# janelia-flyem/transfer_em

Hardware: AMD Instinct MI355X
Metric: CycleGAN train steps/sec on 132^3 x1 uint8 volumes (per-GPU batch of 1 volume; aggregate over GPUs) (higher is better)
Workload: dtype f32

## Files before the change

include/tem_hip.h:

```cpp
#ifndef TEM_HIP_H
#define TEM_HIP_H

#include <stdint.h>

#ifdef __cplusplus
extern "C" {
#endif

#define TEM_ABI_VERSION 1

#define TEM_OK            0
#define TEM_EINVAL       -1
#define TEM_EUNSUPPORTED -2
#define TEM_ESHAPE       -3

typedef void *tem_stream_t;

typedef struct tem_view {
  float  *ptr;
  int32_t N, D, H, W, C;
  int64_t sN, sD, sH, sW;
} tem_view;

typedef struct tem_epilogue {
// ... 94 lines not shown
int tem_adam_keras(float *theta, const float *grad, float *m, float *v, int64_t n,
                   float lr, float beta1, float beta2, float eps, float grad_scale,
                   const uint32_t *step_dev, tem_stream_t stream);

int tem_step_tick(uint32_t *step_dev, tem_stream_t stream);

int tem_dropout_masks(uint8_t *mask0, int64_t nbytes0, uint32_t site0, uint8_t *mask1, int64_t nbytes1, uint32_t site1,
                      uint64_t seed, const uint32_t *step_dev, uint32_t step, tem_stream_t stream);

int tem_u8_to_f32_std(const uint8_t *in, float *out, int64_t n, float mean, float std,
                      tem_stream_t stream);

int tem_f32_unstd_to_u8(const tem_view *y, uint8_t *out, int64_t oD, int64_t oH, int64_t oW,
                        float mean, float std, tem_stream_t stream);

int tem_u8_tiles_to_f32_std(const uint8_t *vol, int32_t Z, int32_t Y, int32_t X, const int32_t *origins_dev,
                            int32_t ntile, int32_t edge, float *out, float mean, float std, tem_stream_t stream);

int tem_f32_tiles_unstd_to_u8(const float *y, int32_t ntile, int32_t yedge, int32_t tpad, const int32_t *index_dev,
                              uint8_t *out, int32_t OZ, int32_t OY, int32_t OX, float mean, float std,
                              tem_stream_t stream);

int tem_augment_f32(const float *src, int32_t D, int32_t H, int32_t W, int32_t p0, int32_t p1, int32_t p2,
                    int32_t f0, int32_t f1, int32_t f2, float scale, float shift, float *dst, tem_stream_t stream);

int tem_warp_f32(const float *src, int32_t D, int32_t H, int32_t W, float rate, uint64_t seed, float *dst,
                 uint8_t *seeds, double *sum, tem_stream_t stream);

int tem_fill_f32(float *dst, int64_t n, float value, tem_stream_t stream);

int tem_copy_view(const tem_view *src, const tem_view *dst, tem_stream_t stream);

int tem_add_view(const tem_view *src, const tem_view *dst, tem_stream_t stream);

typedef struct tem_wlayer {
  int64_t offset;
  int32_t ntap, ci, co;
} tem_wlayer;

int tem_flip_transpose(const float *theta, float *theta_t, const tem_wlayer *layers_dev, int32_t nlayers,
                       int64_t total, tem_stream_t stream);

typedef struct tem_wino_layer {
  int64_t src_off, dst_off;
  int32_t ci, co, flip;
} tem_wino_layer;

int tem_winograd_weights(const float *theta, float *u, const tem_wino_layer *layers_dev, int32_t nlayers,
                         tem_stream_t stream);

int tem_conv_bwd_weight_winograd_nslab(const tem_bww_args *a, char *name, int32_t name_len);
int tem_conv_bwd_weight_winograd(const tem_bww_args *a, tem_stream_t stream);

int tem_leaky_gate_view(const tem_view *g, const tem_view *saved, float slope, tem_stream_t stream);

int tem_conv_bf16(const tem_conv_args *a, tem_stream_t stream);

int tem_conv_bf16_describe(const tem_conv_args *a, char *name, int32_t name_len);

int tem_conv_transpose_bf16(const tem_conv_args *a, tem_stream_t stream);
int tem_conv_transpose_bf16_describe(const tem_conv_args *a, char *name, int32_t name_len);

int tem_conv_bwd_weight_bf16(const tem_bww_args *a, tem_stream_t stream);
int tem_conv_bwd_weight_bf16_nslab(const tem_bww_args *a, char *name, int32_t name_len);

int tem_cast_f32_to_bf16(const float *src, void *dst, int64_t n, tem_stream_t stream);

int tem_pack_weights_bf16(const float *theta, void *theta_h, void *theta_ht, const tem_wlayer *layers_dev,
                          int32_t nlayers, int64_t total, tem_stream_t stream);

int tem_focal_logits_bf16(const tem_view *z, int32_t target, float gamma, double *losses, uint32_t slot_mask,
                          float loss_scale, const tem_view *dz, float grad_scale, tem_stream_t stream);
int tem_focal_match_bf16(const tem_view *a, const tem_view *b, float gamma, double *losses, uint32_t slot_mask,
                         float loss_scale, const tem_view *db, float grad_scale, tem_stream_t stream);
int tem_copy_view_bf16(const tem_view *src, const tem_view *dst, tem_stream_t stream);
int tem_add_view_bf16(const tem_view *src, const tem_view *dst, tem_stream_t stream);
int tem_channel_sum_bf16(const tem_view *g, float *out, int32_t accumulate, tem_stream_t stream);

int tem_instance_norm(const tem_view *x, const float *scale, const float *offset, float eps,
                      const tem_view *y, float *mean, float *rstd, tem_stream_t stream);

int tem_instance_norm_bwd(const tem_view *x, const tem_view *dy, const float *scale, const float *mean,
                          const float *rstd, const tem_view *dx, float *dscale, float *doffset,
                          double *workspace, tem_stream_t stream);

int tem_abi_version(const char **arch);

#ifdef __cplusplus
}
#endif
#endif
```

transfer_em_amd/_lib.py:

```python
import ctypes as C
import os

import torch

_HERE = os.path.dirname(os.path.abspath(__file__))
LIB_PATH = os.path.join(_HERE, "lib", "libtem_hip.so")

TEM_OK, TEM_EINVAL, TEM_EUNSUPPORTED, TEM_ESHAPE = 0, -1, -2, -3
TEM_W_TAP_CI_CO, TEM_W_FLIP_CO_CI, TEM_W_WINOGRAD = 0, 1, 2
_ERR = {TEM_EINVAL: "TEM_EINVAL (malformed descriptor)",
        TEM_EUNSUPPORTED: "TEM_EUNSUPPORTED (geometry outside the compiled set)",
        TEM_ESHAPE: "TEM_ESHAPE (inconsistent tensor extents)"}


class TemError(RuntimeError):
    pass


class tem_view(C.Structure):
    _fields_ = [("ptr", C.c_void_p),
                ("N", C.c_int32), ("D", C.c_int32), ("H", C.c_int32), ("W", C.c_int32), ("C", C.c_int32),
                ("sN", C.c_int64), ("sD", C.c_int64), ("sH", C.c_int64), ("sW", C.c_int64)]


# ... 40 lines not shown

_VP = C.POINTER(tem_view)
_SIGS = {
    "tem_disc_head_nslab": [C.c_int64],
    "tem_disc_head_fwd": [C.c_void_p, C.c_void_p, C.c_void_p, C.c_void_p, C.c_void_p, C.c_void_p, C.c_int64, C.c_float, C.c_void_p],
    "tem_disc_head_bwd": [C.POINTER(tem_head_bwd_args), C.c_void_p],
    "tem_conv": [C.POINTER(tem_conv_args), C.c_void_p],
    "tem_conv_transpose": [C.POINTER(tem_conv_args), C.c_void_p],
    "tem_conv_direct": [C.POINTER(tem_conv_args), C.c_void_p],
    "tem_conv_transpose_direct": [C.POINTER(tem_conv_args), C.c_void_p],
    "tem_conv_bf16": [C.POINTER(tem_conv_args), C.c_void_p],
    "tem_conv_bf16_describe": [C.POINTER(tem_conv_args), C.c_char_p, C.c_int32],
    "tem_conv_transpose_bf16": [C.POINTER(tem_conv_args), C.c_void_p],
    "tem_conv_transpose_bf16_describe": [C.POINTER(tem_conv_args), C.c_char_p, C.c_int32],
    "tem_conv_bwd_weight_bf16": [C.POINTER(tem_bww_args), C.c_void_p],
    "tem_conv_bwd_weight_bf16_nslab": [C.POINTER(tem_bww_args), C.c_char_p, C.c_int32],
    "tem_cast_f32_to_bf16": [C.c_void_p, C.c_void_p, C.c_int64, C.c_void_p],
    "tem_pack_weights_bf16": [C.c_void_p, C.c_void_p, C.c_void_p, C.c_void_p, C.c_int32, C.c_int64, C.c_void_p],
    "tem_focal_logits_bf16": [_VP, C.c_int32, C.c_float, C.c_void_p, C.c_uint32, C.c_float, _VP, C.c_float, C.c_void_p],
    "tem_focal_match_bf16": [_VP, _VP, C.c_float, C.c_void_p, C.c_uint32, C.c_float, _VP, C.c_float, C.c_void_p],
    "tem_copy_view_bf16": [_VP, _VP, C.c_void_p],
    "tem_add_view_bf16": [_VP, _VP, C.c_void_p],
    "tem_channel_sum_bf16": [_VP, C.c_void_p, C.c_int32, C.c_void_p],
    "tem_conv_is_tiled": [C.POINTER(tem_conv_args), C.c_int32, C.c_char_p, C.c_int32],
    "tem_bww_is_tiled": [C.POINTER(tem_bww_args), C.c_char_p, C.c_int32],
    "tem_conv_bwd_weight": [C.POINTER(tem_bww_args), C.c_void_p],
    "tem_conv_bwd_weight_nslab": [C.POINTER(tem_bww_args)],
    "tem_reduce_slabs": [C.c_void_p, C.c_int32, C.c_int64, C.c_int64, C.c_void_p, C.c_int32, C.c_float, C.c_void_p],
    "tem_reduce_slabs_multi": [C.c_void_p, C.c_int32, C.c_float, C.c_void_p],
    "tem_channel_sum": [_VP, C.c_void_p, C.c_int32, C.c_void_p],
    "tem_focal_logits": [_VP, C.c_int32, C.c_float, C.c_void_p, C.c_uint32, C.c_float, _VP, C.c_float, C.c_void_p],
    "tem_focal_match": [_VP, _VP, C.c_float, C.c_void_p, C.c_uint32, C.c_float, _VP, C.c_float, C.c_void_p],
    "tem_adam_keras": [C.c_void_p, C.c_void_p, C.c_void_p, C.c_void_p, C.c_int64, C.c_float, C.c_float, C.c_float,
                       C.c_float, C.c_float, C.c_void_p, C.c_void_p],
    "tem_step_tick": [C.c_void_p, C.c_void_p],
    "tem_dropout_masks": [C.c_void_p, C.c_int64, C.c_uint32, C.c_void_p, C.c_int64, C.c_uint32, C.c_uint64, C.c_void_p,
                          C.c_uint32, C.c_void_p],
    "tem_u8_to_f32_std": [C.c_void_p, C.c_void_p, C.c_int64, C.c_float, C.c_float, C.c_void_p],
    "tem_f32_unstd_to_u8": [_VP, C.c_void_p, C.c_int64, C.c_int64, C.c_int64, C.c_float, C.c_float, C.c_void_p],
    "tem_u8_tiles_to_f32_std": [C.c_void_p, C.c_int32, C.c_int32, C.c_int32, C.c_void_p, C.c_int32, C.c_int32, C.c_void_p,
                                C.c_float, C.c_float, C.c_void_p],
    "tem_f32_tiles_unstd_to_u8": [C.c_void_p, C.c_int32, C.c_int32, C.c_int32, C.c_void_p, C.c_void_p, C.c_int32, C.c_int32,
                                  C.c_int32, C.c_float, C.c_float, C.c_void_p],
    "tem_augment_f32": [C.c_void_p, C.c_int32, C.c_int32, C.c_int32, C.c_int32, C.c_int32, C.c_int32, C.c_int32, C.c_int32,
                        C.c_int32, C.c_float, C.c_float, C.c_void_p, C.c_void_p],
    "tem_warp_f32": [C.c_void_p, C.c_int32, C.c_int32, C.c_int32, C.c_float, C.c_uint64, C.c_void_p, C.c_void_p, C.c_void_p,
                     C.c_void_p],
    "tem_fill_f32": [C.c_void_p, C.c_int64, C.c_float, C.c_void_p],
    "tem_copy_view": [_VP, _VP, C.c_void_p],
    "tem_add_view": [_VP, _VP, C.c_void_p],
    "tem_leaky_gate_view": [_VP, _VP, C.c_float, C.c_void_p],
    "tem_flip_transpose": [C.c_void_p, C.c_void_p, C.c_void_p, C.c_int32, C.c_int64, C.c_void_p],
    "tem_conv_bwd_weight_winograd_nslab": [C.POINTER(tem_bww_args), C.c_char_p, C.c_int32],
    "tem_conv_bwd_weight_winograd": [C.POINTER(tem_bww_args), C.c_void_p],
    "tem_winograd_weights": [C.c_void_p, C.c_void_p, C.c_void_p, C.c_int32, C.c_void_p],
    "tem_instance_norm": [_VP, C.c_void_p, C.c_void_p, C.c_float, _VP, C.c_void_p, C.c_void_p, C.c_void_p],
    "tem_instance_norm_bwd": [_VP, _VP, C.c_void_p, C.c_void_p, C.c_void_p, _VP, C.c_void_p, C.c_void_p, C.c_void_p,
                              C.c_void_p],
    "tem_abi_version": [C.POINTER(C.c_char_p)],
}
EXPORTS = tuple(_SIGS)

_lib = None


def load():
    global _lib
    if _lib is not None:
        return _lib
    if not os.path.exists(LIB_PATH):
        raise TemError(
            f"{LIB_PATH} not found: the HIP extension is not built. Run `python -c 'import __graft_entry__ as g; "
            "g.build()'` (or `python -m transfer_em_amd.build`). transfer_em_amd has no CPU fallback.")
    lib = C.CDLL(LIB_PATH)
    for name, argtypes in _SIGS.items():
        try:
            fn = getattr(lib, name)
        except AttributeError as e:
            raise TemError(f"libtem_hip.so does not export {name}; rebuild it") from e
        fn.argtypes = argtypes
        fn.restype = C.c_int
    _lib = lib
    return lib


def check(rc, what):
    if rc != 0:
        msg = _ERR.get(rc, f"hipError {rc}")
        raise TemError(f"{what}: {msg}")
```

transfer_em_amd/csrc/wino.hip:

```cpp
#include "tem_common.h"
#include "wino_common.h"
#include <cmath>
#include <cstdio>
#include <cstdlib>

namespace wino {

#ifdef TEM_DEBUG_KNOBS
#define KDBG(x) (x)
#else
#define KDBG(x) 0
#endif


struct Ep32 {
  float slope;
  const float *gate; int32_t gN, gD, gH, gW; float gate_slope;
  const uint8_t *keep_mask;
  int32_t doz, doy, dox, dD, dH, dW;
  int32_t gbytes, mbytes;
};

struct Dev {
  const float *in0, *in1;
  int32_t i0N, i0D, i0H, i0W, i1N, i1D, i1H, i1W;
  int32_t C0;
  int32_t N, D, H, W;
  const float *u;
  float *out0, *out1;
  int32_t o0N, o0D, o0H, o0W, o1N, o1D, o1H, o1W;
  int32_t CO0;
  int32_t OD, OH, OW;
  int32_t P;
  int32_t BY, BX, nby, nbx, zsegs, zper, NTZ;
  int32_t E, PLC, subb, slotb;
  int32_t ndma;
  int32_t span0, span1;
  uint32_t magicBX, magicE;
  int32_t dbg;
  int32_t obytes;
  unsigned long long *stamps;
  Ep32 ep;
};

template <int CI, int CO, int NI, int EP, int EE>
__global__ __launch_bounds__(512) void wino_conv_k(Dev p) {
  constexpr int NH = CI / 8, VB = 32;
  constexpr int NB = (CO + 15) / 16;
  constexpr bool STREAM = CI == 32;
  constexpr bool PAIR = CI == 8 && CO == 8;
  constexpr int NKZ = PAIR ? 4 : 3;
  constexpr int UCH = 2 * NB * 16 * 128;
  extern __shared__ __attribute__((aligned(16))) float lds[];
  char *const ring = reinterpret_cast<char *>(lds);
  const int tid = threadIdx.x, lane = tid & 63;
  const int wave = __builtin_amdgcn_readfirstlane(tid >> 6);
  const int m = lane & 15, q = lane >> 4;
  const int grp = PAIR ? wave : (NB == 1 ? wave >> 1 : wave >> 2);
  const int nb = NB == 1 ? 0 : (wave >> 1) & 1;
  const int zb = PAIR ? (q >> 1) : (wave & 1);
  const int co = PAIR ? 4 * (q & 1) : nb * 16 + 4 * q;
  float *const uld = reinterpret_cast<float *>(ring + 4 * p.slotb);

  int seg = (int)xcd_contiguous_block(blockIdx.x, gridDim.x);
  const int zseg = seg % p.zsegs; seg /= p.zsegs;
  const int bx = seg % p.nbx; seg /= p.nbx;
  const int by = seg % p.nby;
  const int n = seg / p.nby;
  const int tz0 = zseg * p.zper, tz1 = min(p.NTZ, tz0 + p.zper), nsteps = tz1 - tz0;
  const int oy0 = by * 2 * p.BY, ox0 = bx * 2 * p.BX;
  const int ntile = p.BY * p.BX;

  const bool two_in = p.in1 != p.in0;
  const float *const in0n = p.in0 + (size_t)n * p.i0N, *const in1n = p.in1 + (size_t)n * p.i1N;
  int voff0[NI], voff1[NI];
  {
    const int iy0 = oy0 - p.P, ix0 = ox0 - p.P;
#pragma unroll
    for (int i = 0; i < NI; ++i) {
      const int sp = (wave + 8 * i) * 64 + lane;
      const bool ex = sp < p.PLC;
      const int spc = ex ? sp : 0;
      const int cpos = spc & 1, ve = spc >> 1;
      const int ro = ve / EE, e = ve - ro * EE;
      const int o = ro & 1, yr = ro >> 1;
      const int c = (cpos ^ swz(e, yr)) * 4;
      const int iy = iy0 + yr, ix = ix0 + 2 * e + o;
      const bool ok = ex && (unsigned)iy < (unsigned)p.H && (unsigned)ix < (unsigned)p.W;
      voff0[i] = ok ? (iy * p.i0H + ix * p.i0W + c) * 4 : (int)0x80000000;
      voff1[i] = ok ? (iy * p.i1H + ix * p.i1W + c) * 4 : (int)0x80000000;
      asm volatile("" : "+v"(voff0[i]), "+v"(voff1[i]));
    }
  }
  auto dma_plane = [&](int iz, int slot) {
    const bool zok = (unsigned)iz < (unsigned)p.D;
    const int izc = zok ? iz : 0;
#pragma unroll
    for (int h = 0; h < NH; ++h) {
      char *const dst = ring + slot * p.slotb + h * p.subb;
      if (!two_in || 8 * h < p.C0)
        dma_subimage<NI, !STREAM>(in0n + izc * p.i0D + 8 * h, zok ? p.span0 - 32 * h : 0, voff0, dst, wave, p.ndma);
      else
        dma_subimage<NI, !STREAM>(in1n + izc * p.i1D + (8 * h - p.C0), zok ? p.span1 - 4 * (8 * h - p.C0) : 0, voff1, dst, wave, p.ndma);
    }
  };

  const int izb0 = 2 * tz0 - p.P;
  if (nsteps > 0) {
#pragma unroll
    for (int k = 0; k < 4; ++k) dma_plane(izb0 + k, k);
  }
  auto dma_u = [&](int chunk, int buf) {
    const __amdgpu_buffer_rsrc_t r = __builtin_amdgcn_make_buffer_rsrc((void *)(p.u + (size_t)chunk * UCH), 0, UCH * 4, 0x00020000);
#pragma unroll
    for (int i = 0; i < UCH * 4 / 1024 / 8; ++i) {
      const int j = wave + 8 * i;
      __builtin_amdgcn_raw_ptr_buffer_load_lds(r, (__attribute__((address_space(3))) void *)((char *)uld + buf * (UCH * 4) + j * 1024), 16,
                                               (j * 64 + lane) * 16, 0, 0, 0);
    }
  };
  if (STREAM) {
    dma_u(0, 0);
  } else {
    constexpr int UF4 = NKZ * NH * NB * 16 * 64 * 2 / 4;
    static_assert(UF4 % 512 == 0, "whole 1 KB wave transfers");
    const __amdgpu_buffer_rsrc_t ur = __builtin_amdgcn_make_buffer_rsrc((void *)p.u, 0, UF4 * 16, 0x00020000);
#pragma unroll
    for (int i = 0; i < UF4 / 512; ++i) {
      const int j = wave + 8 * i;
      __builtin_amdgcn_raw_ptr_buffer_load_lds(ur, (__attribute__((address_space(3))) void *)((char *)uld + j * 1024), 16,
                                               (j * 64 + lane) * 16, 0, 0, 0);
    }
  }
  asm volatile("s_waitcnt vmcnt(0)" ::: "memory");
  __syncthreads();

  constexpr int rowb = EE * VB;
  const Ep32 &ep = p.ep;
  float *const out0n = p.out0 + (size_t)n * p.o0N, *const out1n = EP == 2 ? p.out1 + (size_t)n * p.o1N : nullptr;
  const float *const gaten = EP >= 1 ? ep.gate + (size_t)n * ep.gN : nullptr;
  const bool in0c = EP != 2 || co < p.CO0;
  float *const obase = EP == 2 ? (in0c ? out0n : out1n) : out0n;
  const int oco = in0c ? co : co - p.CO0;
  const int oD = in0c ? p.o0D : p.o1D, oH = in0c ? p.o0H : p.o1H, oW = in0c ? p.o0W : p.o1W;
  const __amdgpu_buffer_rsrc_t grs = __builtin_amdgcn_make_buffer_rsrc((void *)gaten, 0, EP >= 1 ? ep.gbytes : 0, 0x00020000);
  const __amdgpu_buffer_rsrc_t mrs = __builtin_amdgcn_make_buffer_rsrc((void *)ep.keep_mask, 0, EP == 2 ? ep.mbytes : 0, 0x00020000);
  const int mpv = EP == 2 ? p.CO0 >> 3 : 0;
  const int kshift = co & 4;
  int gso[4], mso[4], oso[4];
#pragma unroll
  for (int o4 = 0; o4 < 4; ++o4) {
    gso[o4] = EP >= 1 ? ((o4 >> 1) * ep.gH + (o4 & 1) * ep.gW) * 4 : 0;
    mso[o4] = EP == 2 ? ((o4 >> 1) * ep.dW + (o4 & 1)) * mpv : 0;
    oso[o4] = ((o4 >> 1) * p.o0H + (o4 & 1) * p.o0W) * 4;
  }
  const __amdgpu_buffer_rsrc_t ors = __builtin_amdgcn_make_buffer_rsrc((void *)out0n, 0, EP != 2 ? p.obytes : 0, 0x00020000);

  const int tA = min(grp * 16 + m, ntile - 1);
  const int tyA = (int)fdiv((uint32_t)tA, (uint32_t)p.BX, p.magicBX), txA = tA - tyA * p.BX;
  const int a0 = (4 * tyA * EE + txA) * VB + (q & 1) * 8;
  int cs[2][2];
#pragma unroll
  for (int a = 0; a < 2; ++a)
#pragma unroll
    for (int b = 0; b < 2; ++b) cs[a][b] = ((q >> 1) ^ swz(txA + a, 2 * (tyA + b))) * 16;

#ifdef TEM_DEBUG_KNOBS
  unsigned long long t_last = p.stamps ? clock64() : 0, t_sum[8] = {0, 0, 0, 0, 0, 0, 0, 0};
#define STAMP(i) do { if (p.stamps) { unsigned long long t_now = clock64(); t_sum[i] += t_now - t_last; t_last = t_now; } } while (0)
#else
#define STAMP(i) do { } while (0)
#endif
  f32x4 acc[16];
  f32x4 gv[4];
  uint32_t kb[4];
  uint32_t tyx, tok4 = 0;
  {
    const int t = grp * 16 + m;
    const int ty = (int)fdiv((uint32_t)t, (uint32_t)p.BX, p.magicBX), tx = t - ty * p.BX;
    const int oy = oy0 + 2 * ty, ox = ox0 + 2 * tx;
    const bool tok = co < CO && t < ntile;
#pragma unroll
    for (int o4 = 0; o4 < 4; ++o4) tok4 |= ((tok && oy + (o4 >> 1) < p.OH && ox + (o4 & 1) < p.OW) ? 1u : 0u) << o4;
    tyx = ((uint32_t)oy << 16) | (uint32_t)ox;
  }
  auto tile_geom = [&](int oz, int &o0, int &go, int &mb, uint32_t &okm) {
    uint32_t yx = tyx;
    asm volatile("" : "+v"(yx));
    const int oy = (int)(yx >> 16), ox = (int)(yx & 0xffffu);
    okm = oz < p.OD ? tok4 : 0u;
    o0 = oz * oD + oy * oH + ox * oW + oco;
    go = EP >= 1 ? (oz * ep.gD + oy * ep.gH + ox * ep.gW + co) * 4 : 0;
    mb = EP == 2 ? (int)(((((uint32_t)n * ep.dD + (oz + ep.doz)) * ep.dH + (oy + ep.doy)) * ep.dW + (ox + ep.dox)) * (uint32_t)mpv) + (co >> 3) : 0;
  };
  auto fetch_ep = [&](int oz) {
    int o0, go, mb;
    uint32_t okm;
    tile_geom(oz, o0, go, mb, okm);
    if (!in0c) okm = 0;
#pragma unroll
    for (int o4 = 0; o4 < 4; ++o4) {
      const bool okf = (okm >> o4) & 1u;
      int goff = okf ? go : (int)0x80000000;
      asm volatile("" : "+v"(goff));
      const u32x4 g4 = __builtin_amdgcn_raw_buffer_load_b128(grs, goff, gso[o4], 0);
      gv[o4] = f32x4{__uint_as_float(g4.x), __uint_as_float(g4.y), __uint_as_float(g4.z), __uint_as_float(g4.w)};
      if (EP == 2) {
        int moff = okf ? mb : (int)0x80000000;
        asm volatile("" : "+v"(moff));
        kb[o4] = (uint32_t)__builtin_amdgcn_raw_buffer_load_b8(mrs, moff, mso[o4], 0) >> kshift;
      }
    }
  };
  auto finish = [&](int oz) {
    f32x4 yx[4][2], yy[2][2];
#pragma unroll
    for (int a = 0; a < 4; ++a) at4(acc[a * 4 + 0], acc[a * 4 + 1], acc[a * 4 + 2], acc[a * 4 + 3], yx[a][0], yx[a][1]);
#pragma unroll
    for (int b = 0; b < 2; ++b) at4(yx[0][b], yx[1][b], yx[2][b], yx[3][b], yy[0][b], yy[1][b]);
    int o0, go, mb;
    uint32_t okm;
    tile_geom(oz, o0, go, mb, okm);
#pragma unroll
    for (int o4 = 0; o4 < 4; ++o4) {
      const bool ok = (okm >> o4) & 1u;
      f32x4 val = yy[o4 >> 1][o4 & 1];
#pragma unroll
      for (int r = 0; r < 4; ++r) {
        if (EP == 0) val[r] = fmaxf(val[r], ep.slope * val[r]);
        if (EP >= 1 && in0c) {
          val[r] = gv[o4][r] > 0.f ? val[r] : ep.gate_slope * val[r];
          if (EP == 2) val[r] = ((kb[o4] >> r) & 1u) ? 2.f * val[r] : 0.f;
        }
      }
      if (EP == 2 || STREAM) {
        if (ok) *reinterpret_cast<f32x4 *>(obase + o0 + (o4 >> 1) * oH + (o4 & 1) * oW) = val;
      } else {
        int so = ok ? o0 * 4 + oso[o4] : (int)0x80000000;
        asm volatile("" : "+v"(so));
        __builtin_amdgcn_raw_buffer_store_b128(u32x4{__float_as_uint(val[0]), __float_as_uint(val[1]), __float_as_uint(val[2]), __float_as_uint(val[3])},
                                               ors, so, 0, 0);
      }
    }
  };

  for (int step = 0; step < nsteps; ++step) {
    const int tz = tz0 + step, oz = 2 * tz + zb, izb = 2 * tz - p.P;
    const bool more = step + 1 < nsteps;
    const int sA = (step & 1) ? 2 : 0;
    STAMP(0);
    if (EP >= 1) fetch_ep(oz);

#pragma unroll
    for (int i = 0; i < 16; ++i) acc[i] = f32x4{0.f, 0.f, 0.f, 0.f};
#pragma unroll
    for (int kz = 0; kz < NKZ; ++kz) {
      const int pl = PAIR ? kz : zb + kz;
      const char *plane = ring + ((pl < 2 ? sA : 2 - sA) + (pl & 1)) * p.slotb + a0;
#pragma unroll
      for (int h = 0; h < NH; ++h) {
        f32x2 v[4][4];
#pragma unroll
        for (int dy = 0; dy < 4; ++dy)
#pragma unroll
          for (int dx = 0; dx < 4; ++dx)
            v[dy][dx] = *reinterpret_cast<const f32x2 *>(plane + h * p.subb + (2 * dy + (dx & 1)) * rowb + (dx >> 1) * VB + cs[dx >> 1][dy >> 1]);
        if (kz == 1 && h == NH - 1) {
          __syncthreads();
          if (more && !(KDBG(p.dbg & 4))) { dma_plane(izb + 4, sA); dma_plane(izb + 5, sA + 1); }
        }
#pragma unroll
        for (int a = 0; a < 4; ++a) bt4(v[a][0], v[a][1], v[a][2], v[a][3]);
#pragma unroll
        for (int b = 0; b < 4; ++b) bt4(v[0][b], v[1][b], v[2][b], v[3][b]);
        if (STREAM && !(h & 1)) {
          const int c = kz * 2 + (h >> 1);
          if (c > 0) __syncthreads();
          if (c < 5) dma_u(c + 1, (c + 1) & 1);
          else if (more) dma_u(0, 0);
        }
        const float *uh = STREAM ? uld + ((kz * 2 + (h >> 1)) & 1) * UCH + (((h & 1) * NB + nb) * 16) * 128 + lane * 2
                                 : uld + (((kz * NH + h) * NB + nb) * 16) * 128 + lane * 2;
        f32x2 uf[16];
#pragma unroll
        for (int pt = 0; pt < 16; ++pt) uf[pt] = *reinterpret_cast<const f32x2 *>(uh + pt * 128);
#pragma unroll
        for (int pt = 0; pt < 16; ++pt) acc[pt] = __builtin_amdgcn_mfma_f32_16x16x4f32(uf[pt].x, v[pt >> 2][pt & 3].x, acc[pt], 0, 0, 0);
#pragma unroll
        for (int pt = 0; pt < 16; ++pt) acc[pt] = __builtin_amdgcn_mfma_f32_16x16x4f32(uf[pt].y, v[pt >> 2][pt & 3].y, acc[pt], 0, 0, 0);
      }
    }
    STAMP(1);

    finish(oz);
    STAMP(3);
    asm volatile("s_waitcnt vmcnt(0)" ::: "memory");
    __syncthreads();
  }
  static_assert(!PAIR || EP <= 1, "8 -> 8: forward and gated input-gradient only");

#ifdef TEM_DEBUG_KNOBS
  if (p.stamps && lane == 0) {
    for (int i = 0; i < 8; ++i) p.stamps[((size_t)blockIdx.x * 8 + wave) * 8 + i] = t_sum[i];
  }
#endif
#undef STAMP
}

__global__ __launch_bounds__(256) void wino_weights_k(const float *theta, float *u, const tem_wino_layer *layers) {
  const tem_wino_layer L = layers[blockIdx.x];
  const int nb = blockIdx.z, NB = (L.co + 15) / 16;
  const int co = nb * 16 + (threadIdx.x & 15), ci = (threadIdx.x >> 4) + 16 * blockIdx.y;
  if (ci >= L.ci || nb >= NB) return;
  const int NH = L.ci / 8;
  const bool pair = L.ci == 8 && L.co == 8;
  const int h = ci >> 3, q = (ci & 7) >> 1, j = ci & 1;
  if (pair) {
    if (nb) return;
    const int c16 = threadIdx.x & 15, s_ = c16 >> 3, c8 = c16 & 7;
    auto g4p = [](float a, float b, float c, float (&o)[4]) {
      o[0] = a; o[1] = 0.5f * (a + b + c); o[2] = 0.5f * (a - b + c); o[3] = c;
    };
    for (int pl = 0; pl < 4; ++pl) {
      const int kz = pl - s_;
      float gy[4][4];
      if (kz >= 0 && kz <= 2) {
        float g[3][3], gx[3][4];
        for (int t9 = 0; t9 < 9; ++t9) {
          const int t = kz * 9 + t9;
          g[t9 / 3][t9 % 3] = L.flip ? theta[L.src_off + ((int64_t)(26 - t) * 8 + c8) * 8 + ci] : theta[L.src_off + ((int64_t)t * 8 + ci) * 8 + c8];
        }
        for (int a = 0; a < 3; ++a) g4p(g[a][0], g[a][1], g[a][2], gx[a]);
        for (int x = 0; x < 4; ++x) {
          float o[4];
          g4p(gx[0][x], gx[1][x], gx[2][x], o);
          for (int y = 0; y < 4; ++y) gy[y][x] = o[y];
        }
      } else {
        for (int y = 0; y < 4; ++y) for (int x = 0; x < 4; ++x) gy[y][x] = 0.f;
      }
      float *d = u + L.dst_off + ((int64_t)(pl * 16) * 64 + (q * 16 + c16)) * 2 + j;
      for (int pt = 0; pt < 16; ++pt) d[pt * 128] = gy[pt >> 2][pt & 3];
    }
    return;
  }
  auto g4 = [](float a, float b, float c, float (&o)[4]) {
    o[0] = a; o[1] = 0.5f * (a + b + c); o[2] = 0.5f * (a - b + c); o[3] = c;
  };
#pragma unroll
  for (int kz = 0; kz < 3; ++kz) {
    float g[3][3];
#pragma unroll
    for (int t9 = 0; t9 < 9; ++t9) {
      const int t = kz * 9 + t9;
      float w = 0.f;
      if (co < L.co) w = L.flip ? theta[L.src_off + ((int64_t)(26 - t) * L.co + co) * L.ci + ci]
                                : theta[L.src_off + ((int64_t)t * L.ci + ci) * L.co + co];
      g[t9 / 3][t9 % 3] = w;
    }
    float gx[3][4], gy[4][4];
#pragma unroll
    for (int a = 0; a < 3; ++a) g4(g[a][0], g[a][1], g[a][2], gx[a]);
#pragma unroll
    for (int x = 0; x < 4; ++x) {
      float o[4];
      g4(gx[0][x], gx[1][x], gx[2][x], o);
#pragma unroll
      for (int y = 0; y < 4; ++y) gy[y][x] = o[y];
    }
    float *d = u + L.dst_off + ((int64_t)(((kz * NH + h) * NB + nb) * 16) * 64 + (q * 16 + (co & 15))) * 2 + j;
#pragma unroll
    for (int pt = 0; pt < 16; ++pt) d[pt * 128] = gy[pt >> 2][pt & 3];
  }
}

constexpr int LDS_MAX = 160 * 1024;
static thread_local char *g_name = nullptr;
static thread_local int g_name_len = 0;

template <int CI, int CO, int NI>
int plan(Dev &p, double *cost, size_t *lds_bytes, int EE) {
  constexpr int NH = CI / 8, NB = (CO + 15) / 16;
  constexpr bool PAIR = CI == 8 && CO == 8;
  const size_t ubytes = CI == 32 ? (size_t)2 * (2 * NB * 16 * 128) * 4
                                 : (size_t)(PAIR ? 4 : 3) * NH * NB * 16 * 64 * 2 * 4;
  const int TY = (p.OH + 1) / 2, TX = (p.OW + 1) / 2;
  double best = 1e300;
  static const int knob_cus = tem_env_int("TEM_WINO_CUS", 256), knob_cuw = tem_env_int("TEM_WINO_CUW", 400);
  for (int by = 1; by <= TY && by <= 64; ++by)
    for (int bx = 1; bx <= TX && bx <= 64; ++bx) {
      const int nt = by * bx;
      if (nt > (PAIR ? 128 : 64 / NB)) continue;
      if (bx + 1 > EE) continue;
      const int E = EE, plv = (2 * by + 2) * 2 * E;
      const int subb = (plv * 32 + 1023) & ~1023, slotb = NH * subb;
      const size_t bytes = (size_t)4 * slotb + ubytes;
      const int ndma = subb / 1024;
      if (bytes > (size_t)LDS_MAX || ndma > 8 * NI) continue;
      const int nby = (TY + by - 1) / by, nbx = (TX + bx - 1) / bx;
      const int cols = p.N * nby * nbx;
      const int wraps = (16 % bx) ? 1 : 0;
      const double step = 2.0 * (PAIR ? 4 : 3) * NH * 32 * 45.0 * (1.0 + 0.03 * wraps) + 3500.0 + (CI == 32 ? 3000.0 : 0.0);
      const double pro = 6000.0 + (4.0 * slotb + ubytes) / 10.0;
      for (int zs = 1; zs <= p.NTZ; ++zs) {
        const int zper = (p.NTZ + zs - 1) / zs, zsegs = (p.NTZ + zper - 1) / zper;
        if (zsegs != zs) continue;
        const double t = std::ceil(cols * zsegs / (double)knob_cus) * (pro + zper * step) +
                         knob_cuw / 100.0 * (cols * zsegs / 256.0) * (pro + zper * step);
        if (t < best) {
          best = t; p.BY = by; p.BX = bx; p.nby = nby; p.nbx = nbx; p.zsegs = zsegs; p.zper = zper;
          p.E = E; p.PLC = plv * 2; p.subb = subb; p.slotb = slotb; p.ndma = ndma; *lds_bytes = (bytes + 15) & ~(size_t)15;
        }
      }
    }
  *cost = best;
  return best < 1e300 ? TEM_OK : TEM_EUNSUPPORTED;
}

template <int CI, int CO, int NI>
int plan_memo(Dev &p, double *cost, size_t *lds_bytes, int EE) {
  struct R { int rc, BY, BX, nby, nbx, zsegs, zper, E, PLC, subb, slotb, ndma; size_t lds; double cost; };
  static tem_plan_cache<5, R> cache;
  const std::array<int, 5> key{p.N, p.OH, p.OW, p.NTZ, EE};
  R r;
  if (!cache.get(key, r)) {
    r.lds = 0; r.cost = 1e300;
    r.rc = plan<CI, CO, NI>(p, &r.cost, &r.lds, EE);
    r.BY = p.BY; r.BX = p.BX; r.nby = p.nby; r.nbx = p.nbx; r.zsegs = p.zsegs; r.zper = p.zper; r.E = p.E; r.PLC = p.PLC;
    r.subb = p.subb; r.slotb = p.slotb; r.ndma = p.ndma;
    cache.put(key, r);
  } else {
    p.BY = r.BY; p.BX = r.BX; p.nby = r.nby; p.nbx = r.nbx; p.zsegs = r.zsegs; p.zper = r.zper; p.E = r.E; p.PLC = r.PLC;
    p.subb = r.subb; p.slotb = r.slotb; p.ndma = r.ndma;
  }
  *cost = r.cost; *lds_bytes = r.lds;
  return r.rc;
}

template <int CI, int CO, int NI, int EP, int EE>
static int launch(const Dev &p, size_t lds_bytes, hipStream_t st) {
  const int nblocks = p.N * p.nby * p.nbx * p.zsegs;
  auto kern = wino_conv_k<CI, CO, NI, EP, EE>;
  static bool attr_set = false;
  if (!attr_set) {
    hipError_t e = hipFuncSetAttribute((const void *)kern, hipFuncAttributeMaxDynamicSharedMemorySize, LDS_MAX);
    if (e != hipSuccess) return (int)e;
    attr_set = true;
  }
  hipLaunchKernelGGL(kern, dim3(nblocks), dim3(512), lds_bytes, st, p);
  TEM_CHECK_LAUNCH();
  return TEM_OK;
}

template <int CI, int CO, int NI, int EP>
int run_best(Dev p, hipStream_t st, bool dry) {
  static int force = -1;
  if (force < 0) force = tem_env_int("TEM_WINO_EE", 0);
  const int pitches[2] = {9, 17};
  Dev best = p;
  double cbest = 1e300;
  size_t lds_bytes = 0;
  for (int i = 0; i < 2; ++i) {
    if (force && pitches[i] != force) continue;
    Dev q = p;
    double c = 1e300;
    size_t l = 0;
    if (plan_memo<CI, CO, NI>(q, &c, &l, pitches[i]) == TEM_OK && c < cbest) { best = q; cbest = c; lds_bytes = l; }
  }
  if (cbest >= 1e300) return TEM_EUNSUPPORTED;
  p = best;
  p.magicBX = magic_for(p.BX); p.magicE = magic_for(p.E);
  if (dry) {
    if (g_name) snprintf(g_name, g_name_len, "wino_conv_k<%d, %d, %d, %d, %d>", CI, CO, NI, EP, p.E);
    return TEM_OK;
  }
  const int nblocks = p.N * p.nby * p.nbx * p.zsegs;
  if (KDBG(p.dbg & 8))
    fprintf(stderr, "wino<%d,%d,%d> O=%dx%dx%d: BY=%d BX=%d nby=%d nbx=%d zsegs=%d zper=%d blocks=%d lds=%zu\n", CI, CO, EP,
            p.OD, p.OH, p.OW, p.BY, p.BX, p.nby, p.nbx, p.zsegs, p.zper, nblocks, lds_bytes);
  return p.E == 9 ? launch<CI, CO, NI, EP, 9>(p, lds_bytes, st) : launch<CI, CO, NI, EP, 17>(p, lds_bytes, st);
}

int dispatch(const tem_conv_args *a, hipStream_t st, bool dry) {
  const tem_view &i0 = a->in0, &o0 = a->out0;
  const bool cube = a->kd == 3 && a->kh == 3 && a->kw == 3 && a->sd == 1 && a->sh == 1 && a->sw == 1 && a->pd == a->ph &&
                    a->ph == a->pw;
  if (!cube || a->w_layout != TEM_W_WINOGRAD || a->pd < 0) return TEM_EUNSUPPORTED;
  if (!fits32(i0) || !fits32(o0)) return TEM_EUNSUPPORTED;
  Dev p{};
  p.in0 = i0.ptr; p.i0N = (int)i0.sN; p.i0D = (int)i0.sD; p.i0H = (int)i0.sH; p.i0W = (int)i0.sW; p.C0 = i0.C;
  p.in1 = i0.ptr; p.i1N = p.i0N; p.i1D = p.i0D; p.i1H = p.i0H; p.i1W = p.i0W;
  int CI = i0.C;
  auto aligned = [](const tem_view &v) {
    return ((uintptr_t)v.ptr & 15) == 0 && v.sW % 4 == 0 && v.sH % 4 == 0 && v.sD % 4 == 0 && v.sN % 4 == 0 && v.C % 4 == 0;
  };
  if (!aligned(i0)) return TEM_EUNSUPPORTED;
  if (a->in1.ptr) {
    const tem_view &i1 = a->in1;
    if (i1.N != i0.N || i1.D != i0.D || i1.H != i0.H || i1.W != i0.W) return TEM_ESHAPE;
    if (!fits32(i1) || !aligned(i1)) return TEM_EUNSUPPORTED;
    p.in1 = i1.ptr; p.i1N = (int)i1.sN; p.i1D = (int)i1.sD; p.i1H = (int)i1.sH; p.i1W = (int)i1.sW;
    CI += i1.C;
    if (i0.C % 8) return TEM_EUNSUPPORTED;
  }
  p.N = i0.N; p.D = i0.D; p.H = i0.H; p.W = i0.W;
  p.span0 = (int)(((int64_t)(i0.H - 1) * p.i0H + (int64_t)(i0.W - 1) * p.i0W + i0.C) * 4);
  p.span1 = a->in1.ptr ? (int)(((int64_t)(i0.H - 1) * p.i1H + (int64_t)(i0.W - 1) * p.i1W + a->in1.C) * 4) : p.span0;
  p.u = a->w;
  p.out0 = o0.ptr; p.o0N = (int)o0.sN; p.o0D = (int)o0.sD; p.o0H = (int)o0.sH; p.o0W = (int)o0.sW; p.CO0 = o0.C;
  {
    const int64_t ospan = (int64_t)(o0.D - 1) * o0.sD + (int64_t)(o0.H - 1) * o0.sH + (int64_t)(o0.W - 1) * o0.sW + o0.C;
    if (ospan >= ((int64_t)1 << 29)) return TEM_EUNSUPPORTED;
    p.obytes = (int)(ospan * 4);
  }
  int CO = o0.C;
  if (a->out1.ptr) {
    const tem_view &o1 = a->out1;
    if (o1.N != o0.N || o1.D != o0.D || o1.H != o0.H || o1.W != o0.W) return TEM_ESHAPE;
    if (!fits32(o1)) return TEM_EUNSUPPORTED;
    p.out1 = o1.ptr; p.o1N = (int)o1.sN; p.o1D = (int)o1.sD; p.o1H = (int)o1.sH; p.o1W = (int)o1.sW;
    CO += o1.C;
  }
  if (o0.N != i0.N) return TEM_ESHAPE;
  if (o0.D != i0.D + 2 * a->pd - 2 || o0.H != i0.H + 2 * a->ph - 2 || o0.W != i0.W + 2 * a->pw - 2) return TEM_ESHAPE;
  p.OD = o0.D; p.OH = o0.H; p.OW = o0.W;
  p.NTZ = (p.OD + 1) / 2;
  p.P = a->pd;
  {
    static int dbg = -1;
    if (dbg < 0) dbg = tem_env_int("TEM_DEBUG_FLAGS", 0);
    p.dbg = dbg;
    static unsigned long long stamp_ptr = ~0ull;
    if (stamp_ptr == ~0ull) stamp_ptr = tem_env_hex("TEM_WINO_STAMP_BUF");
// ... 7 lines not shown
  int EP = 0;
  if (e.gate.ptr) {
    const tem_view &g = e.gate;
    if (g.N != o0.N || g.D != o0.D || g.H != o0.H || g.W != o0.W || g.C < o0.C) return TEM_ESHAPE;
    if (!fits32(g) || e.slope != 1.f) return TEM_EUNSUPPORTED;
    q.gate = g.ptr; q.gN = (int)g.sN; q.gD = (int)g.sD; q.gH = (int)g.sH; q.gW = (int)g.sW;
    const int64_t gspan = (int64_t)(g.D - 1) * g.sD + (int64_t)(g.H - 1) * g.sH + (int64_t)(g.W - 1) * g.sW + g.C;
    if (gspan >= ((int64_t)1 << 29)) return TEM_EUNSUPPORTED;
    q.gbytes = (int)(gspan * 4);
    EP = 1;
  }
  if (e.dropout || a->out1.ptr) {
    if (!(e.dropout && e.keep_mask && e.keep_mode == 2 && a->out1.ptr && EP == 1)) return TEM_EUNSUPPORTED;
    q.keep_mask = e.keep_mask;
    q.doz = e.drop_org[0]; q.doy = e.drop_org[1]; q.dox = e.drop_org[2];
    q.dD = e.drop_dims[0] ? e.drop_dims[0] : o0.D; q.dH = e.drop_dims[0] ? e.drop_dims[1] : o0.H;
    q.dW = e.drop_dims[0] ? e.drop_dims[2] : o0.W;
    if ((int64_t)o0.N * q.dD * q.dH * q.dW * o0.C >= ((int64_t)1 << 32)) return TEM_EUNSUPPORTED;
    if (o0.C % 8) return TEM_EUNSUPPORTED;
    q.mbytes = (int)(((int64_t)o0.N * q.dD * q.dH * q.dW * o0.C + 7) / 8);
    EP = 2;
  }
#define WINO_CASE(ci, co, ni, epi) if (CI == ci && CO == co && EP == epi) return run_best<ci, co, ni, epi>(p, st, dry);
  WINO_CASE(16, 16, 2, 0) WINO_CASE(16, 16, 2, 1) WINO_CASE(16, 16, 2, 2)
  WINO_CASE(8, 8, 3, 0) WINO_CASE(8, 8, 3, 1)
  WINO_CASE(8, 16, 2, 0) WINO_CASE(8, 16, 2, 1)
  WINO_CASE(16, 8, 2, 0) WINO_CASE(16, 8, 2, 1)
  WINO_CASE(16, 32, 2, 0) WINO_CASE(16, 32, 2, 1)
  WINO_CASE(32, 32, 2, 0) WINO_CASE(32, 32, 2, 1) WINO_CASE(32, 32, 2, 2)
  WINO_CASE(32, 16, 2, 0) WINO_CASE(32, 16, 2, 1)
#undef WINO_CASE
  return TEM_EUNSUPPORTED;
}

}

int tem_conv_wino_try(const tem_conv_args *a, hipStream_t st, bool dry) { return wino::dispatch(a, st, dry); }

int tem_conv_wino_describe(const tem_conv_args *a, char *buf, int len) {
  wino::g_name = buf; wino::g_name_len = len;
  int rc = wino::dispatch(a, nullptr, true);
  wino::g_name = nullptr;
  return rc;
}

extern "C" int tem_winograd_weights(const float *theta, float *u, const tem_wino_layer *layers_dev, int32_t nlayers,
                                    tem_stream_t stream) {
  TEM_CLEAR_ERR();
  if (!theta || !u || !layers_dev || nlayers <= 0) return TEM_EINVAL;
  hipLaunchKernelGGL(wino::wino_weights_k, dim3(nlayers, 2, 2), dim3(256), 0, (hipStream_t)stream, theta, u, layers_dev);
  TEM_CHECK_LAUNCH();
  return TEM_OK;
}
```

Before: 122.1.

## Make Winograd conv kernel persistent with chained work items and cross-item prefetch

Turns the Winograd 3x3x3 conv kernel into a persistent kernel. It launches at most 256 workgroups, and each one walks a contiguous range of (column, z-segment) items. While finishing the current item it prefetches the input planes and weights of the next one, which hides per-block prologue and launch tail costs. The planner gains a separate cost model for persistent mode with tunable gap and weight knobs. This adds register pressure and kernarg reloads, and persistent mode is enabled by default only for the eligible template variants.

After: 122.2, median of 6. No clear change (+0.0%).

```diff
diff --git a/include/tem_hip.h b/include/tem_hip.h
--- a/include/tem_hip.h
+++ b/include/tem_hip.h
@@ -170,6 +170,8 @@
 int tem_conv_bwd_weight_winograd_nslab(const tem_bww_args *a, char *name, int32_t name_len);
 int tem_conv_bwd_weight_winograd(const tem_bww_args *a, tem_stream_t stream);
 
+int tem_wino_persistent(int32_t mode);
+
 int tem_leaky_gate_view(const tem_view *g, const tem_view *saved, float slope, tem_stream_t stream);
 
 int tem_conv_bf16(const tem_conv_args *a, tem_stream_t stream);
diff --git a/transfer_em_amd/_lib.py b/transfer_em_amd/_lib.py
--- a/transfer_em_amd/_lib.py
+++ b/transfer_em_amd/_lib.py
@@ -116,6 +116,7 @@
     "tem_leaky_gate_view": [_VP, _VP, C.c_float, C.c_void_p],
     "tem_flip_transpose": [C.c_void_p, C.c_void_p, C.c_void_p, C.c_int32, C.c_int64, C.c_void_p],
     "tem_conv_bwd_weight_winograd_nslab": [C.POINTER(tem_bww_args), C.c_char_p, C.c_int32],
+    "tem_wino_persistent": [C.c_int32],
     "tem_conv_bwd_weight_winograd": [C.POINTER(tem_bww_args), C.c_void_p],
     "tem_winograd_weights": [C.c_void_p, C.c_void_p, C.c_void_p, C.c_int32, C.c_void_p],
     "tem_instance_norm": [_VP, C.c_void_p, C.c_void_p, C.c_float, _VP, C.c_void_p, C.c_void_p, C.c_void_p],
diff --git a/transfer_em_amd/csrc/wino.hip b/transfer_em_amd/csrc/wino.hip
--- a/transfer_em_amd/csrc/wino.hip
+++ b/transfer_em_amd/csrc/wino.hip
@@ -33,6 +33,7 @@
   int32_t OD, OH, OW;
   int32_t P;
   int32_t BY, BX, nby, nbx, zsegs, zper, NTZ;
+  int32_t nitems;
   int32_t E, PLC, subb, slotb;
   int32_t ndma;
   int32_t span0, span1;
@@ -43,11 +44,14 @@
   Ep32 ep;
 };
 
+constexpr bool walks(int ci, int ep) { return ep == 0 || ci == 32; }
+
 template <int CI, int CO, int NI, int EP, int EE>
 __global__ __launch_bounds__(512) void wino_conv_k(Dev p) {
   constexpr int NH = CI / 8, VB = 32;
   constexpr int NB = (CO + 15) / 16;
   constexpr bool STREAM = CI == 32;
+  constexpr bool WALK = walks(CI, EP);
   constexpr bool PAIR = CI == 8 && CO == 8;
   constexpr int NKZ = PAIR ? 4 : 3;
   constexpr int UCH = 2 * NB * 16 * 128;
@@ -62,20 +66,38 @@
   const int co = PAIR ? 4 * (q & 1) : nb * 16 + 4 * q;
   float *const uld = reinterpret_cast<float *>(ring + 4 * p.slotb);
 
-  int seg = (int)xcd_contiguous_block(blockIdx.x, gridDim.x);
-  const int zseg = seg % p.zsegs; seg /= p.zsegs;
-  const int bx = seg % p.nbx; seg /= p.nbx;
-  const int by = seg % p.nby;
-  const int n = seg / p.nby;
-  const int tz0 = zseg * p.zper, tz1 = min(p.NTZ, tz0 + p.zper), nsteps = tz1 - tz0;
-  const int oy0 = by * 2 * p.BY, ox0 = bx * 2 * p.BX;
+  typedef __attribute__((address_space(4))) const Dev KDev;
+  auto kargs = []() -> KDev & {
+    KDev *k = (KDev *)__builtin_amdgcn_kernarg_segment_ptr();
+    asm volatile("" : "+s"(k));
+    return *k;
+  };
+  const int pos = (int)xcd_contiguous_block(blockIdx.x, gridDim.x);
+  const int ipw = p.nitems / (int)gridDim.x, irem = p.nitems - ipw * (int)gridDim.x;
+  const int it0 = pos * ipw + min(pos, irem), it1 = it0 + ipw + (pos < irem ? 1 : 0);
+  int n, oy0, ox0, tz0, nsteps, itn;
+  auto run_at = [&](int it, int &n_, int &oy0_, int &ox0_, int &tz0_, int &nsteps_, int &itn_) {
+    KDev &p = kargs();
+    const int col = it / p.zsegs;
+    int c = col;
+    const int bx = c % p.nbx; c /= p.nbx;
+    const int by = c % p.nby;
+    n_ = c / p.nby;
+    oy0_ = by * 2 * p.BY; ox0_ = bx * 2 * p.BX;
+    itn_ = min(it1, (col + 1) * p.zsegs);
+    tz0_ = (it - col * p.zsegs) * p.zper;
+    nsteps_ = min(p.NTZ, (itn_ - col * p.zsegs) * p.zper) - tz0_;
+  };
+  run_at(it0, n, oy0, ox0, tz0, nsteps, itn);
   const int ntile = p.BY * p.BX;
 
   const bool two_in = p.in1 != p.in0;
-  const float *const in0n = p.in0 + (size_t)n * p.i0N, *const in1n = p.in1 + (size_t)n * p.i1N;
+  auto opaque_n = [](int v) { asm volatile("" : "+s"(v)); return v; };
+  int sn = n;
   int voff0[NI], voff1[NI];
-  {
-    const int iy0 = oy0 - p.P, ix0 = ox0 - p.P;
+  auto make_voff = [&](int oy0_, int ox0_, int (&v0)[NI], int (&v1)[NI]) {
+    KDev &p = kargs();
+    const int iy0 = oy0_ - p.P, ix0 = ox0_ - p.P;
 #pragma unroll
     for (int i = 0; i < NI; ++i) {
       const int sp = (wave + 8 * i) * 64 + lane;
@@ -87,14 +109,17 @@
       const int c = (cpos ^ swz(e, yr)) * 4;
       const int iy = iy0 + yr, ix = ix0 + 2 * e + o;
       const bool ok = ex && (unsigned)iy < (unsigned)p.H && (unsigned)ix < (unsigned)p.W;
-      voff0[i] = ok ? (iy * p.i0H + ix * p.i0W + c) * 4 : (int)0x80000000;
-      voff1[i] = ok ? (iy * p.i1H + ix * p.i1W + c) * 4 : (int)0x80000000;
-      asm volatile("" : "+v"(voff0[i]), "+v"(voff1[i]));
-    }
-  }
+      v0[i] = ok ? (iy * p.i0H + ix * p.i0W + c) * 4 : (int)0x80000000;
+      v1[i] = ok ? (iy * p.i1H + ix * p.i1W + c) * 4 : (int)0x80000000;
+      asm volatile("" : "+v"(v0[i]), "+v"(v1[i]));
+    }
+  };
+  make_voff(oy0, ox0, voff0, voff1);
   auto dma_plane = [&](int iz, int slot) {
     const bool zok = (unsigned)iz < (unsigned)p.D;
     const int izc = zok ? iz : 0;
+    const int n_ = opaque_n(sn);
+    const float *const in0n = p.in0 + (size_t)n_ * p.i0N, *const in1n = p.in1 + (size_t)n_ * p.i1N;
 #pragma unroll
     for (int h = 0; h < NH; ++h) {
       char *const dst = ring + slot * p.slotb + h * p.subb;
@@ -137,13 +162,9 @@
 
   constexpr int rowb = EE * VB;
   const Ep32 &ep = p.ep;
-  float *const out0n = p.out0 + (size_t)n * p.o0N, *const out1n = EP == 2 ? p.out1 + (size_t)n * p.o1N : nullptr;
-  const float *const gaten = EP >= 1 ? ep.gate + (size_t)n * ep.gN : nullptr;
   const bool in0c = EP != 2 || co < p.CO0;
-  float *const obase = EP == 2 ? (in0c ? out0n : out1n) : out0n;
   const int oco = in0c ? co : co - p.CO0;
   const int oD = in0c ? p.o0D : p.o1D, oH = in0c ? p.o0H : p.o1H, oW = in0c ? p.o0W : p.o1W;
-  const __amdgpu_buffer_rsrc_t grs = __builtin_amdgcn_make_buffer_rsrc((void *)gaten, 0, EP >= 1 ? ep.gbytes : 0, 0x00020000);
   const __amdgpu_buffer_rsrc_t mrs = __builtin_amdgcn_make_buffer_rsrc((void *)ep.keep_mask, 0, EP == 2 ? ep.mbytes : 0, 0x00020000);
   const int mpv = EP == 2 ? p.CO0 >> 3 : 0;
   const int kshift = co & 4;
@@ -154,7 +175,7 @@
     mso[o4] = EP == 2 ? ((o4 >> 1) * ep.dW + (o4 & 1)) * mpv : 0;
     oso[o4] = ((o4 >> 1) * p.o0H + (o4 & 1) * p.o0W) * 4;
   }
-  const __amdgpu_buffer_rsrc_t ors = __builtin_amdgcn_make_buffer_rsrc((void *)out0n, 0, EP != 2 ? p.obytes : 0, 0x00020000);
+  auto out0n = [&]() { return p.out0 + (size_t)opaque_n(n) * p.o0N; };
 
   const int tA = min(grp * 16 + m, ntile - 1);
   const int tyA = (int)fdiv((uint32_t)tA, (uint32_t)p.BX, p.magicBX), txA = tA - tyA * p.BX;
@@ -174,16 +195,19 @@
   f32x4 acc[16];
   f32x4 gv[4];
   uint32_t kb[4];
-  uint32_t tyx, tok4 = 0;
-  {
+  uint32_t tyx, tok4;
+  auto set_tile = [&](int oy0_, int ox0_) {
+    KDev &p = kargs();
     const int t = grp * 16 + m;
     const int ty = (int)fdiv((uint32_t)t, (uint32_t)p.BX, p.magicBX), tx = t - ty * p.BX;
-    const int oy = oy0 + 2 * ty, ox = ox0 + 2 * tx;
+    const int oy = oy0_ + 2 * ty, ox = ox0_ + 2 * tx;
     const bool tok = co < CO && t < ntile;
+    tok4 = 0;
 #pragma unroll
     for (int o4 = 0; o4 < 4; ++o4) tok4 |= ((tok && oy + (o4 >> 1) < p.OH && ox + (o4 & 1) < p.OW) ? 1u : 0u) << o4;
     tyx = ((uint32_t)oy << 16) | (uint32_t)ox;
-  }
+  };
+  set_tile(oy0, ox0);
   auto tile_geom = [&](int oz, int &o0, int &go, int &mb, uint32_t &okm) {
     uint32_t yx = tyx;
     asm volatile("" : "+v"(yx));
@@ -198,6 +222,8 @@
     uint32_t okm;
     tile_geom(oz, o0, go, mb, okm);
     if (!in0c) okm = 0;
+    const __amdgpu_buffer_rsrc_t grs = __builtin_amdgcn_make_buffer_rsrc((void *)(ep.gate + (size_t)opaque_n(n) * ep.gN), 0,
+                                                                         EP >= 1 ? ep.gbytes : 0, 0x00020000);
 #pragma unroll
     for (int o4 = 0; o4 < 4; ++o4) {
       const bool okf = (okm >> o4) & 1u;
@@ -234,8 +260,12 @@
         }
       }
       if (EP == 2 || STREAM) {
+        float *b0 = out0n(), *b1 = EP == 2 ? p.out1 + (size_t)opaque_n(n) * p.o1N : b0;
+        asm volatile("" : "+s"(b0), "+s"(b1));
+        float *const obase = in0c ? b0 : b1;
         if (ok) *reinterpret_cast<f32x4 *>(obase + o0 + (o4 >> 1) * oH + (o4 & 1) * oW) = val;
       } else {
+        const __amdgpu_buffer_rsrc_t ors = __builtin_amdgcn_make_buffer_rsrc((void *)out0n(), 0, p.obytes, 0x00020000);
         int so = ok ? o0 * 4 + oso[o4] : (int)0x80000000;
         asm volatile("" : "+v"(so));
         __builtin_amdgcn_raw_buffer_store_b128(u32x4{__float_as_uint(val[0]), __float_as_uint(val[1]), __float_as_uint(val[2]), __float_as_uint(val[3])},
@@ -244,10 +274,14 @@
     }
   };
 
+  int sA = 0;
+  for (;;) {
+  const bool has_next = WALK && itn < it1;
+  int nizb0 = 0;
   for (int step = 0; step < nsteps; ++step) {
     const int tz = tz0 + step, oz = 2 * tz + zb, izb = 2 * tz - p.P;
     const bool more = step + 1 < nsteps;
-    const int sA = (step & 1) ? 2 : 0;
+    const bool chain = !more && has_next;
     STAMP(0);
     if (EP >= 1) fetch_ep(oz);
 
@@ -267,7 +301,16 @@
             v[dy][dx] = *reinterpret_cast<const f32x2 *>(plane + h * p.subb + (2 * dy + (dx & 1)) * rowb + (dx >> 1) * VB + cs[dx >> 1][dy >> 1]);
         if (kz == 1 && h == NH - 1) {
           __syncthreads();
-          if (more && !(KDBG(p.dbg & 4))) { dma_plane(izb + 4, sA); dma_plane(izb + 5, sA + 1); }
+          if (chain) {
+            int nn, noy0, nox0, ntz0, nns, nitn;
+            run_at(itn, nn, noy0, nox0, ntz0, nns, nitn);
+            make_voff(noy0, nox0, voff0, voff1);
+            sn = nn; nizb0 = 2 * ntz0 - kargs().P;
+          }
+          if ((more || chain) && !(KDBG(p.dbg & 4))) {
+            const int iz = more ? izb + 4 : nizb0;
+            dma_plane(iz, sA); dma_plane(iz + 1, sA + 1);
+          }
         }
 #pragma unroll
         for (int a = 0; a < 4; ++a) bt4(v[a][0], v[a][1], v[a][2], v[a][3]);
@@ -277,7 +320,7 @@
           const int c = kz * 2 + (h >> 1);
           if (c > 0) __syncthreads();
           if (c < 5) dma_u(c + 1, (c + 1) & 1);
-          else if (more) dma_u(0, 0);
+          else if (more || chain) dma_u(0, 0);
         }
         const float *uh = STREAM ? uld + ((kz * 2 + (h >> 1)) & 1) * UCH + (((h & 1) * NB + nb) * 16) * 128 + lane * 2
                                  : uld + (((kz * NH + h) * NB + nb) * 16) * 128 + lane * 2;
@@ -291,11 +334,20 @@
       }
     }
     STAMP(1);
+    if (chain) {
+      __syncthreads();
+      dma_plane(nizb0 + 2, 2 - sA); dma_plane(nizb0 + 3, 3 - sA);
+    }
 
     finish(oz);
     STAMP(3);
     asm volatile("s_waitcnt vmcnt(0)" ::: "memory");
     __syncthreads();
+    if (more) sA = 2 - sA;
+  }
+  if (!has_next) break;
+  run_at(itn, n, oy0, ox0, tz0, nsteps, itn);
+  set_tile(oy0, ox0);
   }
   static_assert(!PAIR || EP <= 1, "8 -> 8: forward and gated input-gradient only");
 
@@ -375,11 +427,20 @@
 }
 
 constexpr int LDS_MAX = 160 * 1024;
+
+constexpr int RESIDENT = 256;
+static int persistent_mode() {
+  static int mode = [] { const char *v = getenv("TEM_WINO_PERSISTENT"); return v ? (atoi(v) != 0) : 1; }();
+  return mode;
+}
+static int g_persistent = -1;
+static int persistent() { return g_persistent >= 0 ? g_persistent : persistent_mode(); }
+static void set_persistent(int on) { g_persistent = on != 0; }
 static thread_local char *g_name = nullptr;
 static thread_local int g_name_len = 0;
 
 template <int CI, int CO, int NI>
-int plan(Dev &p, double *cost, size_t *lds_bytes, int EE) {
+int plan(Dev &p, double *cost, size_t *lds_bytes, int EE, bool persist) {
   constexpr int NH = CI / 8, NB = (CO + 15) / 16;
   constexpr bool PAIR = CI == 8 && CO == 8;
   const size_t ubytes = CI == 32 ? (size_t)2 * (2 * NB * 16 * 128) * 4
@@ -387,6 +448,8 @@
   const int TY = (p.OH + 1) / 2, TX = (p.OW + 1) / 2;
   double best = 1e300;
   static const int knob_cus = tem_env_int("TEM_WINO_CUS", 256), knob_cuw = tem_env_int("TEM_WINO_CUW", 400);
+  static const double knob_gap = tem_env_int("TEM_WINO_GAP", 2000);
+  static const int knob_pcuw = tem_env_int("TEM_WINO_PCUW", 100);
   for (int by = 1; by <= TY && by <= 64; ++by)
     for (int bx = 1; bx <= TX && bx <= 64; ++bx) {
       const int nt = by * bx;
@@ -405,6 +468,18 @@
       for (int zs = 1; zs <= p.NTZ; ++zs) {
         const int zper = (p.NTZ + zs - 1) / zs, zsegs = (p.NTZ + zper - 1) / zper;
         if (zsegs != zs) continue;
+        if (persist) {
+          const int items = cols * zsegs, G = std::min(items, RESIDENT), ipw = (items + G - 1) / G;
+          const int chains = std::min(ipw - 1, (ipw + zsegs - 2) / zsegs + 1);
+          const double busy = pro + ipw * zper * step + chains * knob_gap;
+          const double cut = G * pro + (double)items * zper * step + (double)G * chains * knob_gap;
+          const double t = busy + knob_pcuw / 100.0 * cut / 256.0;
+          if (t < best) {
+            best = t; p.BY = by; p.BX = bx; p.nby = nby; p.nbx = nbx; p.zsegs = zsegs; p.zper = zper;
+            p.E = E; p.PLC = plv * 2; p.subb = subb; p.slotb = slotb; p.ndma = ndma; *lds_bytes = (bytes + 15) & ~(size_t)15;
+          }
+          continue;
+        }
         const double t = std::ceil(cols * zsegs / (double)knob_cus) * (pro + zper * step) +
                          knob_cuw / 100.0 * (cols * zsegs / 256.0) * (pro + zper * step);
         if (t < best) {
@@ -418,14 +493,14 @@
 }
 
 template <int CI, int CO, int NI>
-int plan_memo(Dev &p, double *cost, size_t *lds_bytes, int EE) {
+int plan_memo(Dev &p, double *cost, size_t *lds_bytes, int EE, bool persist) {
   struct R { int rc, BY, BX, nby, nbx, zsegs, zper, E, PLC, subb, slotb, ndma; size_t lds; double cost; };
-  static tem_plan_cache<5, R> cache;
-  const std::array<int, 5> key{p.N, p.OH, p.OW, p.NTZ, EE};
+  static tem_plan_cache<6, R> cache;
+  const std::array<int, 6> key{p.N, p.OH, p.OW, p.NTZ, EE, persist};
   R r;
   if (!cache.get(key, r)) {
     r.lds = 0; r.cost = 1e300;
-    r.rc = plan<CI, CO, NI>(p, &r.cost, &r.lds, EE);
+    r.rc = plan<CI, CO, NI>(p, &r.cost, &r.lds, EE, persist);
     r.BY = p.BY; r.BX = p.BX; r.nby = p.nby; r.nbx = p.nbx; r.zsegs = p.zsegs; r.zper = p.zper; r.E = p.E; r.PLC = p.PLC;
     r.subb = p.subb; r.slotb = p.slotb; r.ndma = p.ndma;
     cache.put(key, r);
@@ -438,8 +513,7 @@
 }
 
 template <int CI, int CO, int NI, int EP, int EE>
-static int launch(const Dev &p, size_t lds_bytes, hipStream_t st) {
-  const int nblocks = p.N * p.nby * p.nbx * p.zsegs;
+static int launch(const Dev &p, int nblocks, size_t lds_bytes, hipStream_t st) {
   auto kern = wino_conv_k<CI, CO, NI, EP, EE>;
   static bool attr_set = false;
   if (!attr_set) {
@@ -457,6 +531,7 @@
   static int force = -1;
   if (force < 0) force = tem_env_int("TEM_WINO_EE", 0);
   const int pitches[2] = {9, 17};
+  const bool persist = persistent() && walks(CI, EP);
   Dev best = p;
   double cbest = 1e300;
   size_t lds_bytes = 0;
@@ -465,20 +540,22 @@
     Dev q = p;
     double c = 1e300;
     size_t l = 0;
-    if (plan_memo<CI, CO, NI>(q, &c, &l, pitches[i]) == TEM_OK && c < cbest) { best = q; cbest = c; lds_bytes = l; }
+    if (plan_memo<CI, CO, NI>(q, &c, &l, pitches[i], persist) == TEM_OK && c < cbest) { best = q; cbest = c; lds_bytes = l; }
   }
   if (cbest >= 1e300) return TEM_EUNSUPPORTED;
   p = best;
   p.magicBX = magic_for(p.BX); p.magicE = magic_for(p.E);
+  p.nitems = p.N * p.nby * p.nbx * p.zsegs;
+  const int nblocks = persist ? std::min(p.nitems, RESIDENT) : p.nitems;
   if (dry) {
-    if (g_name) snprintf(g_name, g_name_len, "wino_conv_k<%d, %d, %d, %d, %d>", CI, CO, NI, EP, p.E);
+    if (g_name) snprintf(g_name, g_name_len, "wino_conv_k<%d, %d, %d, %d, %d> BY=%d BX=%d zper=%d items=%d wgs=%d ipw=%d", CI, CO, NI, EP,
+                         p.E, p.BY, p.BX, p.zper, p.nitems, nblocks, (p.nitems + nblocks - 1) / nblocks);
     return TEM_OK;
   }
-  const int nblocks = p.N * p.nby * p.nbx * p.zsegs;
   if (KDBG(p.dbg & 8))
-    fprintf(stderr, "wino<%d,%d,%d> O=%dx%dx%d: BY=%d BX=%d nby=%d nbx=%d zsegs=%d zper=%d blocks=%d lds=%zu\n", CI, CO, EP,
-            p.OD, p.OH, p.OW, p.BY, p.BX, p.nby, p.nbx, p.zsegs, p.zper, nblocks, lds_bytes);
-  return p.E == 9 ? launch<CI, CO, NI, EP, 9>(p, lds_bytes, st) : launch<CI, CO, NI, EP, 17>(p, lds_bytes, st);
+    fprintf(stderr, "wino<%d,%d,%d> O=%dx%dx%d: BY=%d BX=%d nby=%d nbx=%d zsegs=%d zper=%d items=%d blocks=%d lds=%zu\n", CI, CO, EP,
+            p.OD, p.OH, p.OW, p.BY, p.BX, p.nby, p.nbx, p.zsegs, p.zper, p.nitems, nblocks, lds_bytes);
+  return p.E == 9 ? launch<CI, CO, NI, EP, 9>(p, nblocks, lds_bytes, st) : launch<CI, CO, NI, EP, 17>(p, nblocks, lds_bytes, st);
 }
 
 int dispatch(const tem_conv_args *a, hipStream_t st, bool dry) {
@@ -592,3 +669,9 @@
   TEM_CHECK_LAUNCH();
   return TEM_OK;
 }
+
+extern "C" int tem_wino_persistent(int32_t mode) {
+  const int prev = wino::persistent();
+  if (mode >= 0) wino::set_persistent(mode);
+  return prev;
+}
```
